# adityaX1412/Experiment-YOLO

Measured on AMD Instinct MI355X. Metric: images/sec (train) DEAL-YOLO-N 640x640 bs=64/GPU, higher is better.
Workload: dtype f16; 1 GPU; DEAL-YOLO-N (yolov8n-ASF-P2P2.yaml) train step 640x640, per-GPU batch 64, fwd+TAL/WIOU+NWD/DFL/BCE loss+bwd+SGD+EMA, BASELINE.json configs[1]; loss_mode=wiou+nwd, settle_steps=18, capture_retries=0, global_batch=64, parallelism=dp1, hipgraph=True

## Files before the change

### experiment-yolo_amd/csrc/tensor_ops.hip

```cpp
#include <cstdlib>
#include "common.h"
#include "dealyolo_hip.h"

static inline int grid_for(long total) {
  long b = (total + 255) / 256;
  if (b > 8192) b = 8192;
  if (b < 1) b = 1;
  return (int)b;
}

__global__ __launch_bounds__(256) void import_image_kernel(const float* x, f16* y, int N, int C, int H, int W, int Cp,
                                                           float mul) {
  const long hw = (long)H * W, total = (long)N * hw;
  for (long pix = (long)blockIdx.x * 256 + threadIdx.x; pix < total; pix += (long)gridDim.x * 256) {
    const long n = pix / hw, r = pix - n * hw;
    for (int c0 = 0; c0 < Cp; c0 += 8) {
      half8 v;
#pragma unroll
      for (int j = 0; j < 8; ++j) v[j] = (c0 + j < C) ? (f16)(x[(n * C + c0 + j) * hw + r] * mul) : (f16)0.f;
      *reinterpret_cast<half8*>(y + pix * Cp + c0) = v;
    }
  }
}
extern "C" int dy_import_image(const float* x, void* y, int n, int c, int h, int w, int cp, float mul,
                               hipStream_t stream) {
  if (cp & 7) return DY_ERR_ALIGN;
  hipLaunchKernelGGL(import_image_kernel, dim3(grid_for((long)n * h * w)), dim3(256), 0, stream, x, (f16*)y, n, c, h, w,
                     cp, mul);
  DY_CHECK_LAUNCH();
  return DY_OK;
}

__global__ __launch_bounds__(256) void import_image_u8_kernel(const unsigned char* x, f16* y, long npix, int Cp) {
  const long quads = npix >> 2;
  for (long q = (long)blockIdx.x * 256 + threadIdx.x; q < quads; q += (long)gridDim.x * 256) {
    const unsigned* p = reinterpret_cast<const unsigned*>(x + q * 12);
    const unsigned w0 = p[0], w1 = p[1], w2 = p[2];
    const unsigned char b[12] = {(unsigned char)w0, (unsigned char)(w0 >> 8), (unsigned char)(w0 >> 16), (unsigned char)(w0 >> 24),
                                 (unsigned char)w1, (unsigned char)(w1 >> 8), (unsigned char)(w1 >> 16), (unsigned char)(w1 >> 24),
                                 (unsigned char)w2, (unsigned char)(w2 >> 8), (unsigned char)(w2 >> 16), (unsigned char)(w2 >> 24)};
#pragma unroll
    for (int k = 0; k < 4; ++k) {
      half8 v;
#pragma unroll
      for (int j = 0; j < 8; ++j) v[j] = j < 3 ? (f16)((float)b[3 * k + j] / 255.f) : (f16)0.f;
      f16* d = y + (q * 4 + k) * Cp;
      *reinterpret_cast<half8*>(d) = v;
      for (int c0 = 8; c0 < Cp; c0 += 8) *reinterpret_cast<half8*>(d + c0) = half8{};
    }
  }
  for (long pix = (quads << 2) + (long)blockIdx.x * 256 + threadIdx.x; pix < npix; pix += (long)gridDim.x * 256) {
    half8 v;
#pragma unroll
    for (int j = 0; j < 8; ++j) v[j] = j < 3 ? (f16)((float)x[pix * 3 + j] / 255.f) : (f16)0.f;
    *reinterpret_cast<half8*>(y + pix * Cp) = v;
    for (int c0 = 8; c0 < Cp; c0 += 8) *reinterpret_cast<half8*>(y + pix * Cp + c0) = half8{};
  }
}
static __device__ __forceinline__ void hsv_jitter(float (&c)[3], float r0, float r1, float r2) {
  const float R = c[0], G = c[1], B = c[2];
  const float V = fmaxf(R, fmaxf(G, B)), mn = fminf(R, fminf(G, B)), d = V - mn;
// ... 308 lines not shown
    const long pix = idx / cpp;
    const int c0 = (int)(idx - pix * cpp) * 8;
    const int x0 = (int)(pix % a.W);
    const long t = pix / a.W;
    const int y0 = (int)(t % a.H);
    const long n = t / a.H;
    float s[8];
#pragma unroll
    for (int j = 0; j < 8; ++j) s[j] = 0.f;
    if (a.accumulate) {
      const half8 o = *reinterpret_cast<const half8*>(a.y + pix * a.ldy + c0);
#pragma unroll
      for (int j = 0; j < 8; ++j) s[j] = (float)o[j];
    }
#pragma unroll
    for (int dy = 0; dy < 5; ++dy) {
      const int wy = y0 - (dy - 2);
      const bool yok = wy >= 0 && wy < a.H;
      const int yc = yok ? wy : y0;
      uint2 raw[5];
      half8 g[5];
      bool ok[5];
#pragma unroll
      for (int dx = 0; dx < 5; ++dx) {
        const int wx = x0 - (dx - 2);
        ok[dx] = yok && wx >= 0 && wx < a.W;
        const long wp = (n * a.H + yc) * a.W + (ok[dx] ? wx : x0);
        raw[dx] = *reinterpret_cast<const uint2*>(a.arg + wp * a.C + c0);
        g[dx] = *reinterpret_cast<const half8*>(a.dy + wp * a.lddy + c0);
      }
#pragma unroll
      for (int dx = 0; dx < 5; ++dx) {
        if (!ok[dx]) continue;
        const uint8_t* ai = reinterpret_cast<const uint8_t*>(&raw[dx]);
        const int code = dy * 5 + dx;
#pragma unroll
        for (int j = 0; j < 8; ++j)
          if (ai[j] == code) s[j] += (float)g[dx][j];
      }
    }
    half8 o;
#pragma unroll
    for (int j = 0; j < 8; ++j) o[j] = (f16)s[j];
    *reinterpret_cast<half8*>(a.y + pix * a.ldy + c0) = o;
  }
}
#define SPPF_THREADS 1024
struct SppfArgs {
  f16* cat;
  uint8_t* arg[3];
  int ld, C, N, H, W, acc[3];
};
template <int CG>
__global__ __launch_bounds__(SPPF_THREADS) void sppf_pool3_fwd_kernel(SppfArgs a) {
  constexpr int G = CG / 8;
  extern __shared__ __attribute__((aligned(16))) char sppf_lds[];
  const int HW = a.H * a.W, items = HW * G;
  half8* cur = reinterpret_cast<half8*>(sppf_lds);
  half8* rowm = cur + items;
  uint2* rowa = reinterpret_cast<uint2*>(rowm + items);
  const int groups = a.C / CG, n = blockIdx.x / groups, c0 = (blockIdx.x - n * groups) * CG;
  f16* const base = a.cat + (size_t)n * HW * a.ld + c0;
  for (int i = threadIdx.x; i < items; i += SPPF_THREADS) {
    const int px = i / G, part = i - px * G;
    cur[i] = *reinterpret_cast<const half8*>(base + (size_t)px * a.ld + part * 8);
  }
  __syncthreads();
  for (int l = 0; l < 3; ++l) {
    for (int i = threadIdx.x; i < items; i += SPPF_THREADS) {
      const int px = i / G, part = i - px * G, y = px / a.W, x = px - y * a.W;
      float best[8];
      uint8_t bd[8];
#pragma unroll
      for (int j = 0; j < 8; ++j) { best[j] = -INFINITY; bd[j] = 0; }
#pragma unroll
      for (int dx = 0; dx < 5; ++dx) {
        const int xx = x + dx - 2;
        if (xx < 0 || xx >= a.W) continue;
        const half8 v = cur[(y * a.W + xx) * G + part];
#pragma unroll
        for (int j = 0; j < 8; ++j) {
          const float f = (float)v[j];
          if (f > best[j] || f != f) { best[j] = f; bd[j] = (uint8_t)dx; }
        }
      }
      half8 o;
#pragma unroll
      for (int j = 0; j < 8; ++j) o[j] = (f16)best[j];
      rowm[i] = o;
      rowa[i] = *reinterpret_cast<const uint2*>(bd);
    }
    __syncthreads();
    f16* const yb = base + (size_t)(l + 1) * a.C;
    uint8_t* const ab = a.arg[l] ? a.arg[l] + (size_t)n * HW * a.C + c0 : nullptr;
    for (int i = threadIdx.x; i < items; i += SPPF_THREADS) {
      const int px = i / G, part = i - px * G, y = px / a.W, x = px - y * a.W;
      float best[8];
      uint8_t bi[8];
#pragma unroll
      for (int j = 0; j < 8; ++j) { best[j] = -INFINITY; bi[j] = 0; }
#pragma unroll
      for (int dy = 0; dy < 5; ++dy) {
        const int yy = y + dy - 2;
        if (yy < 0 || yy >= a.H) continue;
        const int k = (yy * a.W + x) * G + part;
        const half8 v = rowm[k];
        const uint2 ra = rowa[k];
        const uint8_t* rd = reinterpret_cast<const uint8_t*>(&ra);
#pragma unroll
        for (int j = 0; j < 8; ++j) {
          const float f = (float)v[j];
          if (f > best[j] || f != f) { best[j] = f; bi[j] = (uint8_t)(dy * 5 + rd[j]); }
        }
      }
      half8 o;
#pragma unroll
      for (int j = 0; j < 8; ++j) o[j] = (f16)best[j];
      cur[i] = o;
      *reinterpret_cast<half8*>(yb + (size_t)px * a.ld + part * 8) = o;
      if (ab) *reinterpret_cast<uint2*>(ab + (size_t)px * a.C + part * 8) = *reinterpret_cast<const uint2*>(bi);
    }
    __syncthreads();
  }
}
template <int CG>
__global__ __launch_bounds__(SPPF_THREADS) void sppf_pool3_bwd_kernel(SppfArgs a) {
  constexpr int G = CG / 8;
  extern __shared__ __attribute__((aligned(16))) char sppf_lds[];
  const int HW = a.H * a.W, items = HW * G;
  half8* g0 = reinterpret_cast<half8*>(sppf_lds);
  half8* g1 = g0 + items;
  uint2* ar = reinterpret_cast<uint2*>(g1 + items);
  const int groups = a.C / CG, n = blockIdx.x / groups, c0 = (blockIdx.x - n * groups) * CG;
  f16* const base = a.cat + (size_t)n * HW * a.ld + c0;
  for (int i = threadIdx.x; i < items; i += SPPF_THREADS) {
    const int px = i / G, part = i - px * G;
    g0[i] = *reinterpret_cast<const half8*>(base + (size_t)3 * a.C + (size_t)px * a.ld + part * 8);
  }
  for (int l = 2; l >= 0; --l) {
    const uint8_t* const ab = a.arg[l] + (size_t)n * HW * a.C + c0;
    for (int i = threadIdx.x; i < items; i += SPPF_THREADS) {
      const int px = i / G, part = i - px * G;
      ar[i] = *reinterpret_cast<const uint2*>(ab + (size_t)px * a.C + part * 8);
    }
    __syncthreads();
    f16* const tb = base + (size_t)l * a.C;
    for (int i = threadIdx.x; i < items; i += SPPF_THREADS) {
      const int px = i / G, part = i - px * G, y = px / a.W, x = px - y * a.W;
      float s[8];
#pragma unroll
      for (int j = 0; j < 8; ++j) s[j] = 0.f;
      if (a.acc[l]) {
        const half8 o = *reinterpret_cast<const half8*>(tb + (size_t)px * a.ld + part * 8);
#pragma unroll
        for (int j = 0; j < 8; ++j) s[j] = (float)o[j];
      }
#pragma unroll
      for (int dy = 0; dy < 5; ++dy) {
        const int wy = y - (dy - 2);
        if (wy < 0 || wy >= a.H) continue;
#pragma unroll
        for (int dx = 0; dx < 5; ++dx) {
          const int wx = x - (dx - 2);
          if (wx < 0 || wx >= a.W) continue;
          const int k = (wy * a.W + wx) * G + part;
          const uint2 raw = ar[k];
          const half8 g = g0[k];
          const uint8_t* ai = reinterpret_cast<const uint8_t*>(&raw);
          const int code = dy * 5 + dx;
#pragma unroll
          for (int j = 0; j < 8; ++j)
            if (ai[j] == code) s[j] += (float)g[j];
        }
      }
      half8 o;
#pragma unroll
      for (int j = 0; j < 8; ++j) o[j] = (f16)s[j];
      if (l > 0) g1[i] = o;
      else *reinterpret_cast<half8*>(tb + (size_t)px * a.ld + part * 8) = o;
    }
    __syncthreads();
    half8* t = g0; g0 = g1; g1 = t;
  }
}
extern "C" int dy_sppf_pool3_supported(int h, int w, int C) {
  if (h < 1 || w < 1 || C < 8 || (C & 7)) return 0;
  const long px = (long)h * w;
  if (!(C & 15) && px * (2 * 32 + 16) <= 156 * 1024) return 16;
  if (px * (2 * 16 + 8) <= 156 * 1024) return 8;
  return 0;
}
extern "C" int dy_sppf_pool3(void* cat, int ld, int C, void* arg0, void* arg1, void* arg2, int n, int h, int w, hipStream_t stream) {
  const int cg = dy_sppf_pool3_supported(h, w, C);
  if (!cg || !cat || ld < 4 * C) return DY_ERR_ARG;
  if ((ld & 7) || ((uintptr_t)cat & 15)) return DY_ERR_ALIGN;
  SppfArgs a{(f16*)cat, {(uint8_t*)arg0, (uint8_t*)arg1, (uint8_t*)arg2}, ld, C, n, h, w, {0, 0, 0}};
  const size_t lds = (size_t)h * w * (cg / 8) * (2 * 16 + 8);
  static bool attr[2] = {false, false};
  if (cg == 16) {
    if (!attr[0]) { if (hipFuncSetAttribute(reinterpret_cast<const void*>(sppf_pool3_fwd_kernel<16>), hipFuncAttributeMaxDynamicSharedMemorySize, 156 * 1024) != hipSuccess) return DY_ERR_LAUNCH; attr[0] = true; }
    hipLaunchKernelGGL(sppf_pool3_fwd_kernel<16>, dim3(n * (C / 16)), dim3(SPPF_THREADS), lds, stream, a);
  } else {
    if (!attr[1]) { if (hipFuncSetAttribute(reinterpret_cast<const void*>(sppf_pool3_fwd_kernel<8>), hipFuncAttributeMaxDynamicSharedMemorySize, 156 * 1024) != hipSuccess) return DY_ERR_LAUNCH; attr[1] = true; }
    hipLaunchKernelGGL(sppf_pool3_fwd_kernel<8>, dim3(n * (C / 8)), dim3(SPPF_THREADS), lds, stream, a);
  }
  DY_CHECK_LAUNCH();
  return DY_OK;
}
extern "C" int dy_sppf_pool3_backward(void* gcat, int ld, int C, const void* arg0, const void* arg1, const void* arg2, int n, int h,
                                      int w, int acc0, int acc1, int acc2, hipStream_t stream) {
  const int cg = dy_sppf_pool3_supported(h, w, C);
  if (!cg || !gcat || !arg0 || !arg1 || !arg2 || ld < 4 * C) return DY_ERR_ARG;
  if ((ld & 7) || ((uintptr_t)gcat & 15)) return DY_ERR_ALIGN;
  SppfArgs a{(f16*)gcat, {(uint8_t*)arg0, (uint8_t*)arg1, (uint8_t*)arg2}, ld, C, n, h, w, {acc0, acc1, acc2}};
  const size_t lds = (size_t)h * w * (cg / 8) * (2 * 16 + 8);
  static bool attr[2] = {false, false};
  if (cg == 16) {
    if (!attr[0]) { if (hipFuncSetAttribute(reinterpret_cast<const void*>(sppf_pool3_bwd_kernel<16>), hipFuncAttributeMaxDynamicSharedMemorySize, 156 * 1024) != hipSuccess) return DY_ERR_LAUNCH; attr[0] = true; }
    hipLaunchKernelGGL(sppf_pool3_bwd_kernel<16>, dim3(n * (C / 16)), dim3(SPPF_THREADS), lds, stream, a);
  } else {
    if (!attr[1]) { if (hipFuncSetAttribute(reinterpret_cast<const void*>(sppf_pool3_bwd_kernel<8>), hipFuncAttributeMaxDynamicSharedMemorySize, 156 * 1024) != hipSuccess) return DY_ERR_LAUNCH; attr[1] = true; }
    hipLaunchKernelGGL(sppf_pool3_bwd_kernel<8>, dim3(n * (C / 8)), dim3(SPPF_THREADS), lds, stream, a);
  }
  DY_CHECK_LAUNCH();
  return DY_OK;
}

extern "C" int dy_maxpool5(const void* x, int ldx, void* y, int ldy, void* argmax, int n, int h, int w, int C,
                           hipStream_t stream) {
  if ((C & 7) || (ldx & 7) || (ldy & 7)) return DY_ERR_ALIGN;
  PoolArgs a{(const f16*)x, (f16*)y, (uint8_t*)argmax, nullptr, ldx, ldy, 0, C, n, h, w, 0};
  hipLaunchKernelGGL(maxpool5_fwd_kernel, dim3(grid_for((long)n * h * w * (C >> 3))), dim3(256), 0, stream, a);
  DY_CHECK_LAUNCH();
  return DY_OK;
}
extern "C" int dy_maxpool5_backward(const void* dy, int lddy, const void* argmax, void* dx, int lddx, int n, int h,
                                    int w, int C, int accumulate, hipStream_t stream) {
  if ((C & 7) || (lddy & 7) || (lddx & 7)) return DY_ERR_ALIGN;
  PoolArgs a{nullptr, (f16*)dx, (uint8_t*)argmax, (const f16*)dy, 0, lddx, lddy, C, n, h, w, accumulate};
  hipLaunchKernelGGL(maxpool5_bwd_kernel, dim3(grid_for((long)n * h * w * (C >> 3))), dim3(256), 0, stream, a);
  DY_CHECK_LAUNCH();
  return DY_OK;
}

struct SsArgs {
  const f16* r[3];
  int ld[3];
  const f16* res;
  int ldres;
// ... 363 lines not shown
          }
        }
        if (a.mode) *reinterpret_cast<half8*>(a.dr[0] + pos * a.lddr[0] + c0) = o;
      }
      half8 o1;
#pragma unroll
      for (int j = 0; j < 8; ++j) {
        const float tot = gs1[j] + (cpp == 4 ? dpp_read<DY_DPP_ROW_SHL(4)>(gs1[j]) : __shfl_xor(gs1[j], cpp, 64));
        const float xh = ((float)own1[j] - mean[j]) * inv[j];
        if (a.mode == 0) {
          if (!(col & 1)) { ps[j] += tot; px[j] += tot * xh; }
        } else {
          o1[j] = (f16)(sc[j] * (tot - 4.f * mg[j] - 4.f * xh * mgx[j]));
        }
      }
      if (a.mode && !(col & 1)) *reinterpret_cast<half8*>(a.dr[1] + lp1 * a.lddr[1] + c0) = o1;
    }
    half8 o2;
#pragma unroll
    for (int j = 0; j < 8; ++j) {
      float tot;
      if (cpp == 4) {
        tot = gs2[j] + dpp_read<DY_DPP_ROW_SHL(4)>(gs2[j]);
        tot += dpp_read<DY_DPP_ROW_SHL(8)>(tot);
      } else {
        tot = gs2[j] + __shfl_xor(gs2[j], cpp, 64);
        tot += __shfl_xor(tot, 2 * cpp, 64);
      }
      const float xh = ((float)own2[j] - mean[j]) * inv[j];
      if (a.mode == 0) {
        if (!(col & 3)) { ps[j] += tot; px[j] += tot * xh; }
      } else {
        o2[j] = (f16)(sc[j] * (tot - 16.f * mg[j] - 16.f * xh * mgx[j]));
      }
    }
    if (a.mode && !(col & 3)) *reinterpret_cast<half8*>(a.dr[2] + lp2 * a.lddr[2] + c0) = o2;
  }
  if (a.mode == 0) {
    __shared__ float red[2][256][9];
    const int rows = 256 / cpp;
#pragma unroll
    for (int j = 0; j < 8; ++j) {
      red[0][tid][j] = ps[j];
      red[1][tid][j] = px[j];
    }
    __syncthreads();
    for (int i = tid; i < 2 * a.C; i += 256) {
      const int which = i / a.C, c = i - which * a.C, pp = c >> 3, j = c & 7;
      float sum = 0.f;
      for (int r = 0; r < rows; ++r) sum += red[which][r * cpp + pp][j];
      a.partials[((size_t)blockIdx.x * 2 + which) * a.C + c] = sum;
    }
  }
}
extern "C" int dy_scalseq_tail_backward_all(const void* r0, int ld0, const void* r1, int ld1, const void* r2, int ld2,
                                            const void* dy, int lddy, void* dr0, int lddr0, void* dr1, int lddr1,
                                            void* dr2, int lddr2, const float* coef, const float* bwdcoef,
                                            float* partials, int max_partials, int n, int h, int w, int C, int mode,
                                            int* nparts, hipStream_t stream) {
  if ((C & 7) || (C >> 3) > 256 || (h & 3) || (w & 3) || (ld0 & 7) || (ld1 & 7) || (ld2 & 7) || (lddy & 7)) return DY_ERR_ARG;
  if (mode && ((lddr0 & 7) || (lddr1 & 7) || (lddr2 & 7) || !dr0 || !dr1 || !dr2 || !bwdcoef)) return DY_ERR_ARG;
  if (!mode && !partials) return DY_ERR_ARG;
  SsBwdAllArgs a{{(const f16*)r0, (const f16*)r1, (const f16*)r2}, {ld0, ld1, ld2}, (const f16*)dy, lddy,
                 {(f16*)dr0, (f16*)dr1, (f16*)dr2}, {lddr0, lddr1, lddr2}, coef, bwdcoef, partials, C, n, h, w, mode};
  const int rows = 256 / (C >> 3);
  long blocks = ((long)n * (h >> 2) * (w >> 2) + rows - 1) / rows;
  if (blocks > 2048) blocks = 2048;
  if (mode == 0 && blocks > max_partials) blocks = max_partials;
  if (blocks < 1) blocks = 1;
  const int cpp = C >> 3;
  if (cpp <= 16 && 64 % cpp == 0 && w % (64 / cpp) == 0) {
    long wblocks = ((long)n * (h >> 2) * (w / (64 / cpp)) + 3) / 4;
    if (wblocks > 2048) wblocks = 2048;
    if (mode == 0 && wblocks > max_partials) wblocks = max_partials;
    if (wblocks < 1) wblocks = 1;
    if (nparts) *nparts = (int)wblocks;
    hipLaunchKernelGGL(scalseq_bwd_cols_kernel, dim3((int)wblocks), dim3(256), 0, stream, a);
    DY_CHECK_LAUNCH();
    return DY_OK;
  }
  if (nparts) *nparts = (int)blocks;
  hipLaunchKernelGGL(scalseq_bwd_all_kernel, dim3((int)blocks), dim3(256), 0, stream, a);
  DY_CHECK_LAUNCH();
  return DY_OK;
}

__global__ __launch_bounds__(256) void copy_slice_kernel(EwArgs e) {
  const int cpp = e.C >> 3;
  const long total = e.npix * cpp;
  for (long idx = (long)blockIdx.x * 256 + threadIdx.x; idx < total; idx += (long)gridDim.x * 256) {
    const long pix = idx / cpp;
    const int c0 = (int)(idx - pix * cpp) * 8;
    *reinterpret_cast<uint4*>(e.y + pix * e.ldy + c0) = *reinterpret_cast<const uint4*>(e.a + pix * e.lda + c0);
  }
}
extern "C" int dy_copy_slice(const void* x, int ldx, void* y, int ldy, long npix, int C, hipStream_t stream) {
  if ((C & 7) || (ldx & 7) || (ldy & 7)) return DY_ERR_ALIGN;
  EwArgs e{(const f16*)x, nullptr, nullptr, (f16*)y, ldx, 0, 0, ldy, C, npix};
  hipLaunchKernelGGL(copy_slice_kernel, dim3(grid_for(npix * (C >> 3))), dim3(256), 0, stream, e);
  DY_CHECK_LAUNCH();
  return DY_OK;
}
extern "C" int dy_fill_zero(void* p, size_t bytes, hipStream_t stream) {
  return hipMemsetAsync(p, 0, bytes, stream) == hipSuccess ? DY_OK : DY_ERR_LAUNCH;
}

struct ZpArgs {
  const f16* x;
  f16* y;
  const f16* dy;
  f16* dx;
  int ldx, ldy, lddy, lddx, C, N, H, W, accumulate;
};
__global__ __launch_bounds__(256) void zoom_pool_fwd_kernel(ZpArgs a) {
  const int cpp = a.C >> 3;
  const long total = (long)a.N * a.H * a.W * cpp;
  for (long idx = (long)blockIdx.x * 256 + threadIdx.x; idx < total; idx += (long)gridDim.x * 256) {
    const long pix = idx / cpp;
    const int c0 = (int)(idx - pix * cpp) * 8;
    const int ox = (int)(pix % a.W);
    const long t = pix / a.W;
    const int oy = (int)(t % a.H);
    const long n = t / a.H;
    float mx[8], sm[8];
#pragma unroll
    for (int i = 0; i < 4; ++i) {
      const long src = (n * 2 * a.H + 2 * oy + (i >> 1)) * 2 * a.W + 2 * ox + (i & 1);
      const half8 v = *reinterpret_cast<const half8*>(a.x + src * a.ldx + c0);
#pragma unroll
// ... 72 lines not shown
```

### experiment-yolo_amd/ultralytics/hip/__init__.py

```python
from __future__ import annotations

import ctypes as C
import os
import sys

_FLAG = "DEBUG_CLR_GRAPH_PACKET_CAPTURE"


def _hip_already_up():
    t = sys.modules.get("torch")
    try:
        return bool(t is not None and t.cuda.is_initialized())
    except Exception:
        return False


if os.environ.get(_FLAG) is None and not _hip_already_up():
    os.environ[_FLAG] = "0"
GRAPH_SAFE = os.environ.get(_FLAG) == "0"

_HERE = os.path.dirname(os.path.abspath(__file__))
LIB_PATH = os.environ.get("DY_HIP_LIB") or os.path.normpath(os.path.join(_HERE, "..", "..", "csrc", "libdealyolo_hip.so"))

DY_EPI_STATS, DY_EPI_BIAS, DY_EPI_SILU, DY_EPI_F32OUT, DY_EPI_ACCUM, DY_EPI_STATS_ACC = 1, 2, 4, 8, 16, 32
# ... 84 lines not shown
    "dy_refine_select": (i32, [vp, vp, vp, vp, vp, i32, C.c_float, C.c_float, vp, vp, vp]),
    "dy_nms_hard": (i32, [vp, vp, vp, i32, C.c_float, vp, vp]),
    "dy_crop_letterbox_u8_multi": (i32, [vp, vp, vp, vp, vp, vp, i32, i32, vp, vp]),
    "dy_refine_select_multi": (i32, [vp, vp, vp, vp, vp, vp, vp, i32, vp, vp, vp]),
    "dy_two_stage_merge": (i32, [vp, vp, vp, vp, vp, vp, i32, f32, vp, vp, f32, i32, vp, vp, vp, vp]),
    "dy_tile_gather_f32": (i32, [vp, vp, vp, vp, vp, vp, vp, i32, i32, vp, vp]),
    "dy_tile_merge": (i32, [vp, vp, vp, vp, vp, i32, i32, i32, f32, i32, i32, vp, vp, vp, vp, vp]),
    "dy_warp_import_u8": (i32, [vp, vp, vp, i32, i32, i32, vp]),
    "dy_warp_slot_bytes": (i32, []),
    "dy_import_image_u8": (i32, [vp, vp, i32, i32, i32, i32, vp, vp, vp, vp]),
    "dy_add": (i32, [vp, i32, vp, i32, vp, i32, vp, i32, i64, i32, vp]),
    "dy_upsample2x": (i32, [vp, i32, vp, i32, i32, i32, i32, i32, i32, i32, vp]),
    "dy_space_to_depth": (i32, [vp, i32, vp, i32, i32, i32, i32, i32, i32, i32, vp]),
    "dy_maxpool5": (i32, [vp, i32, vp, i32, vp, i32, i32, i32, i32, vp]),
    "dy_maxpool5_backward": (i32, [vp, i32, vp, vp, i32, i32, i32, i32, i32, i32, vp]),
    "dy_bn_group_max": (i32, []),
    "dy_bn_act_apply_acc_split": (i32, [vp, i32, vp, i32, vp, i32, i32, vp, vp, vp, vp, vp, vp, i64, i32, i32, f32, f32, f32, vp]),
    "dy_bn_act_bwd_reduce_acc_split": (i32, [vp, i32, vp, i32, i32, vp, i32, vp, vp, i64, i32, i32, vp]),
    "dy_conv1x1_wgrad_bn_planes": (i32, [C.POINTER(DySegs), vp, i32, vp, vp, i32, i32, vp, i32, vp, vp, vp, vp, vp, f32, vp, vp, i32, i32, i32,
                                         i32, i32, i32, vp]),
    "dy_conv1x1_wgrad_dgrad_supported": (i32, [i32, i32, i32, i32, i32]),
    "dy_wgrad_dgrad_kernel_name": (i32, [i32, i32, i32, i32, i32, i32, C.c_char_p, i32]),
    "dy_conv1x1_wgrad_dgrad_bn": (i32, [vp, i32, vp, i32, vp, i32, vp, vp, vp, vp, f32, vp, vp, vp, vp, i32, i32, i32, i32, i32, i32, i32, i32, vp]),
    "dy_conv1x1_wgrad_dgrad_bn_segs": (i32, [C.POINTER(DySegs), vp, i32, vp, i32, vp, vp, vp, vp, f32, vp, vp, vp, C.POINTER(DySegs), i32, i32,
                                             i32, i32, i32, i32, vp]),
    "dy_conv1x1_wgrad_dgrad_bn_planes": (i32, [C.POINTER(DySegs), vp, i32, vp, vp, i32, i32, vp, i32, vp, vp, vp, vp, f32, vp, vp, vp, vp, i32, i32,
                                               C.POINTER(DySegs), i32, i32, i32, i32, i32, i32, vp]),
    "dy_conv1x1_dgrad_bn_supported": (i32, [i32, i32, i32, i32, i32]),
    "dy_dgrad_only_kernel_name": (i32, [i32, i32, i32, i32, i32, i32, C.c_char_p, i32]),
    "dy_conv1x1_dgrad_bn": (i32, [vp, vp, i32, i32, vp, i32, vp, vp, f32, vp, vp, i32, i32, C.POINTER(DySegs), i32, i32, i32, i32, i32, vp]),
    "dy_bn_act_apply_acc_group": (i32, [i32, vp, vp, vp, vp, vp, vp, vp, vp, vp, vp, vp, vp, vp, vp, vp, vp]),
    "dy_bn_act_bwd_reduce_acc_group": (i32, [i32, vp, vp, vp, vp, vp, vp, vp, vp, vp]),
    "dy_bn_act_bwd_reduce_rows": (i32, [vp, i32, vp, i32, vp, vp, i32, i32, i32, i32, vp, i32, i32, vp]),
    "dy_head_box_decode": (i32, [vp, i32, vp, vp, vp, vp, i32, i32, i32, i32, i32, i32, i32, vp]),
    "dy_cls_head_supported": (i32, [i32, i32]),
    "dy_cls_head_slabs": (i32, []),
    "dy_cls_head_forward": (i32, [vp, i32, vp, vp, vp, vp, i64, i32, i32, vp]),
    "dy_cls_head_backward": (i32, [vp, i32, vp, vp, vp, vp, i32, i32, vp, vp, i64, i32, i32, vp]),
    "dy_head_box_decode_levels": (i32, [i32, vp, vp, vp, vp, vp, vp, i32, vp, i32, vp, vp, i32, i32, vp]),
    "dy_conv1x1_rows_backward_levels": (i32, [i32, vp, vp, vp, vp, vp, vp, i32, vp, vp, vp, vp, vp, vp, vp, i32, vp, vp, i32, i32, vp]),
    "dy_cls_head_forward_levels": (i32, [i32, vp, vp, vp, vp, vp, vp, vp, i32, i32, vp]),
    "dy_cls_head_backward_levels": (i32, [i32, vp, vp, vp, vp, vp, vp, vp, vp, vp, vp, vp, i32, i32, vp]),
    "dy_conv1x1_rows_supported": (i32, [i32, i32]),
    "dy_conv1x1_rows_slabs": (i32, [i32, i32, i32]),
    "dy_conv1x1_rows_backward": (i32, [vp, i32, vp, vp, i32, vp, i32, i32, vp, vp, i32, i32, vp, vp, i32, i32, i32, i32, i32, vp]),
    "dy_sppf_pool3_supported": (i32, [i32, i32, i32]),
    "dy_sppf_pool3": (i32, [vp, i32, i32, vp, vp, vp, i32, i32, i32, vp]),
    "dy_sppf_pool3_backward": (i32, [vp, i32, i32, vp, vp, vp, i32, i32, i32, i32, i32, i32, vp]),
    "dy_scalseq_tail": (i32, [vp, i32, vp, i32, vp, i32, vp, i32, vp, i32, vp, i32, i32, i32, i32, vp]),
    "dy_scalseq_tail_backward": (i32, [vp, i32, vp, i32, vp, i32, vp, i32, vp, i32, vp, vp, vp, i32, i32, i32, i32, i32,
                                       i32, i32, ip, vp]),
    "dy_scalseq_tail_backward_all": (i32, [vp, i32, vp, i32, vp, i32, vp, i32, vp, i32, vp, i32, vp, i32, vp, vp, vp, i32, i32,
                                           i32, i32, i32, i32, ip, vp]),
    "dy_zoom_pool": (i32, [vp, i32, vp, i32, i32, i32, i32, i32, vp]),
    "dy_zoom_pool_backward": (i32, [vp, i32, vp, i32, vp, i32, i32, i32, i32, i32, i32, vp]),
    "dy_copy_slice": (i32, [vp, i32, vp, i32, i64, i32, vp]),
    "dy_fill_zero": (i32, [vp, sz, vp]),
    "dy_loss_workspace_bytes": (sz, [i32, i32, i32]),
    "dy_loss_workspace_layout": (i32, [i32, i32, i32, C.POINTER(sz), C.POINTER(sz), C.POINTER(sz)]),
    "dy_detection_loss": (i32, [C.POINTER(DyLossArgs), vp]),
    "dy_tal_assign": (i32, [vp, ip, ip, C.POINTER(f32), i32, i32, i32, i32, i32, vp, vp, vp, vp, vp, vp, vp, vp]),
    "dy_head_infer_supported": (i32, [i32, i32, i32, i32]),
    "dy_head_infer_levels": (i32, [i32, vp, vp, vp, vp, vp, vp, vp, vp, vp, vp, vp, i32, i32, i32, vp, vp]),
    "dy_head_infer_levels_logits": (i32, [i32, vp, vp, vp, vp, vp, vp, vp, vp, vp, vp, vp, i32, i32, i32, vp, vp, vp, vp]),
    "dy_decode_predictions": (i32, [vp, vp, ip, ip, C.POINTER(f32), i32, i32, i32, i32, vp, vp]),
    "dy_nms_candidates": (i32, [vp, i32, i32, i32, f32, i32, vp, i32, vp, vp, vp, vp, i32, vp]),
    "dy_nms_presort_workspace": (sz, [i32, i32]),
    "dy_nms_presort": (i32, [vp, vp, vp, vp, i32, i32, i32, vp, vp, vp, vp, vp]),
    "dy_soft_nms": (i32, [vp, vp, vp, vp, vp, vp, vp, vp, i32, i32, f32, f32, f32, f32, vp]),
    "dy_set_hyper": (i32, [vp, vp, vp]),
    "dy_optimizer_step": (i32, [vp, vp, vp, vp, vp, i64, i64, i64, vp, vp, vp, i64, vp, vp, vp, i32, vp]),
    "dy_optimizer_step_seg": (i32, [vp, vp, vp, vp, vp, i64, lp, vp, vp, vp, i64, vp, vp, vp, i32, vp]),
    "dy_axpy_f32": (i32, [vp, vp, f32, i64, vp]),
    "dy_scale_img": (i32, [vp, i32, i32, i32, i32, i32, i32, i32, i32, vp, vp]),
    "dy_tta_merge": (i32, [i32, C.POINTER(vp), ip, ip, ip, C.POINTER(f32), ip, i32, i32, i32, i32, vp, vp]),
    "dy_bootstrap_ap": (i32, [vp, vp, vp, vp, vp, i32, i32, i32, i32, vp, vp, vp]),
    "dy_confusion_matrix": (i32, [vp, vp, i32, vp, vp, vp, i32, vp, i32, i32, i32, i32, f32, f32, i32, vp, vp, vp]),
    "dy_count_fp": (i32, [vp, vp, vp, vp, vp, i32, f32, C.c_double, vp, vp, vp]),
}

_LIB = None


def lib():
    global _LIB
    if _LIB is None:
        if not os.path.exists(LIB_PATH):
            raise RuntimeError(
                f"{LIB_PATH} not found. The DEAL-YOLO hot path has no CPU/PyTorch fallback: build the HIP library "
                f"first (python -c 'import __graft_entry__ as g; g.build()' or `make -C experiment-yolo_amd/csrc`).")
        L = C.CDLL(LIB_PATH)
        for name, (res, args) in SIGNATURES.items():
            fn = getattr(L, name)
            fn.restype, fn.argtypes = res, args
        if L.dy_segs_bytes() != C.sizeof(DySegs):
            raise RuntimeError(f"{LIB_PATH} lays DySegs out in {L.dy_segs_bytes()} bytes, this binding in {C.sizeof(DySegs)}: rebuild the library")
        if L.dy_loss_args_bytes() != C.sizeof(DyLossArgs):
            raise RuntimeError(f"{LIB_PATH} was built with a DyLossArgs of {L.dy_loss_args_bytes()} bytes, this binding lays out "
                               f"{C.sizeof(DyLossArgs)}: rebuild the library (make -C experiment-yolo_amd/csrc)")
        _LIB = L
    return _LIB


def check(rc, name):
    if rc != 0:
        raise RuntimeError(f"{name} failed: {_ERR.get(rc, rc)}")
# ... 1 lines not shown
```

### include/dealyolo_hip.h

```cpp
#ifndef DEALYOLO_HIP_H
#define DEALYOLO_HIP_H

#include <stddef.h>
#include <stdint.h>

#ifdef __cplusplus
extern "C" {
#endif

#ifndef __HIP__
typedef struct ihipStream_t* hipStream_t;
#endif

#define DY_OK 0
#define DY_ERR_ARG (-1)
#define DY_ERR_LAUNCH (-2)
#define DY_ERR_ALIGN (-3)
#define DY_ERR_CAPACITY (-4)

#define DY_MAX_SEGS 8
typedef struct DySegs {
  int nseg;
  int c_end[DY_MAX_SEGS];
  int ld[DY_MAX_SEGS];
// ... 127 lines not shown
                    int C, int act, hipStream_t stream);
int dy_bn_act_apply_acc(const void* x, int ldx, const void* res, int ldr, void* y, int ldy, const double* acc,
                        const float* gamma, const float* beta, float* running_mean, float* running_var, float* coef,
                        long npix, int C, int act, float count, float eps, float momentum, hipStream_t stream);
int dy_bn_act_bwd_reduce_acc(const void* dy, int lddy, const void* x, int ldx, const float* coef, double* acc, long npix,
                             int C, int act, void* res_grad, int ldrg, int res_accumulate, hipStream_t stream);
int dy_bn_group_max(void);
int dy_bn_act_apply_acc_group(int n, const void* const* x, const int* ldx, void* const* y, const int* ldy, const double* const* acc,
                              const float* const* gamma, const float* const* beta, float* const* running_mean, float* const* running_var,
                              float* const* coef, const long* npix, const int* C, const float* count, const float* eps,
                              const float* momentum, hipStream_t stream);
int dy_bn_act_bwd_reduce_acc_group(int n, const void* const* dy, const int* lddy, const void* const* x, const int* ldx,
                                   const float* const* coef, double* const* acc, const long* npix, const int* C, hipStream_t stream);
int dy_bn_act_bwd_reduce_rows(const void* dy, int lddy, const void* x, int ldx, const float* coef, double* acc, int n, int hw, int C,
                              int act, const int* assigned, int A, int a0, hipStream_t stream);
int dy_bn_act_bwd_apply_acc(const void* dy, int lddy, const void* x, int ldx, void* dx, int lddx, const float* coef,
                            const double* acc, float* dgamma, float* dbeta, long npix, int C, int act, float count,
                            hipStream_t stream);
int dy_bn_act_bwd_reduce(const void* dy, int lddy, const void* x, int ldx, const float* coef, float* partials,
                         int max_partials, long npix, int C, int act, int* nparts, hipStream_t stream);
int dy_bn_bwd_finalize(const float* partials, int nparts, float* dgamma, float* dbeta, float* bwdcoef, int C,
                       float count, int accumulate, hipStream_t stream);
int dy_bn_act_bwd_apply(const void* dy, int lddy, const void* x, int ldx, void* dx, int lddx, const float* coef,
                        const float* bwdcoef, long npix, int C, int act, int frozen_stats, hipStream_t stream);

int dy_import_image(const float* x_nchw, void* y, int n, int c, int h, int w, int cp, float mul, hipStream_t stream);
int dy_import_image_u8(const void* x, void* y, int n, int h, int w, int cp, const void* flip, const int* index,
                       const float* hsv, hipStream_t stream);
int dy_warp_import_u8(const void* pool, const void* slots, void* y, int n, int s, int cp, hipStream_t stream);
int dy_warp_slot_bytes(void);
int dy_add(const void* a, int lda, const void* b, int ldb, const void* c, int ldc, void* y, int ldy, long npix, int C,
           hipStream_t stream);
int dy_upsample2x(const void* x, int ldx, void* y, int ldy, int n, int h, int w, int C, int backward, int accumulate,
                  hipStream_t stream);
int dy_space_to_depth(void* x, int ldx, void* y, int ldy, int n, int h, int w, int C, int backward, int accumulate,
                      hipStream_t stream);
int dy_maxpool5(const void* x, int ldx, void* y, int ldy, void* argmax, int n, int h, int w, int C, hipStream_t stream);
int dy_maxpool5_backward(const void* dy, int lddy, const void* argmax, void* dx, int lddx, int n, int h, int w, int C,
                         int accumulate, hipStream_t stream);
int dy_sppf_pool3_supported(int h, int w, int C);
int dy_sppf_pool3(void* cat, int ld, int C, void* arg0, void* arg1, void* arg2, int n, int h, int w, hipStream_t stream);
int dy_sppf_pool3_backward(void* gcat, int ld, int C, const void* arg0, const void* arg1, const void* arg2, int n, int h, int w,
                           int acc0, int acc1, int acc2, hipStream_t stream);
int dy_scalseq_tail(const void* r0, int ld0, const void* r1, int ld1, const void* r2, int ld2, const void* res,
                    int ldres, void* y, int ldy, const float* coef, int n, int h, int w, int C, hipStream_t stream);
int dy_scalseq_tail_backward(const void* r0, int ld0, const void* r1, int ld1, const void* r2, int ld2, const void* dy,
                             int lddy, void* dr, int lddr, const float* coef, const float* bwdcoef, float* partials,
                             int max_partials, int n, int h, int w, int C, int level, int mode, int* nparts,
                             hipStream_t stream);
int dy_scalseq_tail_backward_all(const void* r0, int ld0, const void* r1, int ld1, const void* r2, int ld2,
                                 const void* dy, int lddy, void* dr0, int lddr0, void* dr1, int lddr1, void* dr2,
                                 int lddr2, const float* coef, const float* bwdcoef, float* partials, int max_partials,
                                 int n, int h, int w, int C, int mode, int* nparts, hipStream_t stream);
int dy_zoom_pool(const void* x, int ldx, void* y, int ldy, int n, int h, int w, int C, hipStream_t stream);
int dy_zoom_pool_backward(const void* x, int ldx, const void* dy, int lddy, void* dx, int lddx, int n, int h, int w, int C,
                          int accumulate, hipStream_t stream);
int dy_copy_slice(const void* x, int ldx, void* y, int ldy, long npix, int C, hipStream_t stream);
int dy_fill_zero(void* p, size_t bytes, hipStream_t stream);

typedef struct DyLossArgs {
  int nl, B, nc, ncp, nmax;
  const float* box[4];
  const float* cls[4];
  void* dbox[4];
  void* dcls[4];
  int H[4], W[4];
  float stride[4];
  const float* t_batch_idx;
  const float* t_cls;
  const float* t_boxes;
  int n_targets;
  const int* n_targets_dev;
  float img_w, img_h;
  float hyp_box, hyp_cls, hyp_dfl;
  int use_wiou, use_nwd;
  float iou_ratio;
  const float* gscale;
  float* scalars;
  void* workspace;
  int dbox_rows_only;
  int box_from_input;
  const void* box_in[4];
  int box_in_ld[4];
  const float* box_w[4];
  const float* box_b[4];
  const float* box_in_coef[4];
  int box_family;
  int box_ltype;
  int box_fm;
  int box_modifier;
  float inner_ratio;
  float focaler_d, focaler_u;
  float shape_scale;
  float piou_lambda;
} DyLossArgs;
#define DY_BOX_FAMILY_LEGACY 0
#define DY_BOX_FAMILY_WISE 1
#define DY_BOX_FAMILY_BBOX 2
#define DY_BOX_IOU 0
#define DY_BOX_WIOU 1
#define DY_BOX_EIOU 2
#define DY_BOX_GIOU 3
#define DY_BOX_DIOU 4
#define DY_BOX_CIOU 5
#define DY_BOX_SIOU 6
#define DY_BOX_SHAPEIOU 7
// ... 115 lines not shown
```

Measured before the change: 6089 images/s.

## Add integer-key SPPF pooling and persistent grid-capped ScalSeq backward kernels

```diff
diff --git a/experiment-yolo_amd/csrc/tensor_ops.hip b/experiment-yolo_amd/csrc/tensor_ops.hip
--- a/experiment-yolo_amd/csrc/tensor_ops.hip
+++ b/experiment-yolo_amd/csrc/tensor_ops.hip
@@ -7,6 +7,10 @@
   if (b > 8192) b = 8192;
   if (b < 1) b = 1;
   return (int)b;
+}
+static bool tensor_ops_v1() {
+  const char* e = getenv("DY_TENSOR_OPS_V1");
+  return e && e[0] == '1' && !e[1];
 }
 
 __global__ __launch_bounds__(256) void import_image_kernel(const float* x, f16* y, int N, int C, int H, int W, int Cp,
@@ -421,9 +425,8 @@
   int ld, C, N, H, W, acc[3];
 };
 template <int CG>
-__global__ __launch_bounds__(SPPF_THREADS) void sppf_pool3_fwd_kernel(SppfArgs a) {
+static __device__ __forceinline__ void sppf_pool3_fwd_body(const SppfArgs& a, char* sppf_lds) {
   constexpr int G = CG / 8;
-  extern __shared__ __attribute__((aligned(16))) char sppf_lds[];
   const int HW = a.H * a.W, items = HW * G;
   half8* cur = reinterpret_cast<half8*>(sppf_lds);
   half8* rowm = cur + items;
@@ -488,6 +491,106 @@
       cur[i] = o;
       *reinterpret_cast<half8*>(yb + (size_t)px * a.ld + part * 8) = o;
       if (ab) *reinterpret_cast<uint2*>(ab + (size_t)px * a.C + part * 8) = *reinterpret_cast<const uint2*>(bi);
+    }
+    __syncthreads();
+  }
+}
+template <int CG>
+__global__ __launch_bounds__(SPPF_THREADS) void sppf_pool3_fwd_kernel(SppfArgs a) {
+  extern __shared__ __attribute__((aligned(16))) char sppf_lds[];
+  sppf_pool3_fwd_body<CG>(a, sppf_lds);
+}
+template <int CG>
+__global__ __launch_bounds__(SPPF_THREADS) void sppf_pool3_fwd_v2_kernel(SppfArgs a) {
+  constexpr int G = CG / 8;
+  constexpr unsigned KNINF = 0x03ffu;
+  extern __shared__ __attribute__((aligned(16))) char sppf_lds[];
+  const int HW = a.H * a.W, items = HW * G;
+  uint4* cur = reinterpret_cast<uint4*>(sppf_lds);
+  uint4* row0 = cur + items;
+  uint4* row1 = row0 + items;
+  int* special = reinterpret_cast<int*>(row1 + items);
+  const int groups = a.C / CG, n = blockIdx.x / groups, c0 = (blockIdx.x - n * groups) * CG;
+  f16* const base = a.cat + (size_t)n * HW * a.ld + c0;
+  if (threadIdx.x == 0) *special = 0;
+  __syncthreads();
+  bool bad = false;
+  for (int i = threadIdx.x; i < items; i += SPPF_THREADS) {
+    const int px = i / G, part = i - px * G;
+    const uint4 v = *reinterpret_cast<const uint4*>(base + (size_t)px * a.ld + part * 8);
+    const unsigned w[4] = {v.x, v.y, v.z, v.w};
+    unsigned k[4];
+#pragma unroll
+    for (int d = 0; d < 4; ++d) {
+      const unsigned lo = w[d] & 0xffffu, hi = w[d] >> 16;
+      bad |= (lo & 0x7fffu) > 0x7c00u || lo == 0x8000u || (hi & 0x7fffu) > 0x7c00u || hi == 0x8000u;
+      k[d] = w[d] ^ ((((w[d] >> 15) & 0x00010001u) * 0xffffu) | 0x80008000u);
+    }
+    cur[i] = uint4{k[0], k[1], k[2], k[3]};
+  }
+  if (bad) *special = 1;
+  __syncthreads();
+  if (*special) {
+    __syncthreads();
+    sppf_pool3_fwd_body<CG>(a, sppf_lds);
+    return;
+  }
+  for (int l = 0; l < 3; ++l) {
+    for (int i = threadIdx.x; i < items; i += SPPF_THREADS) {
+      const int px = i / G, part = i - px * G, y = px / a.W, x = px - y * a.W;
+      unsigned best[8];
+#pragma unroll
+      for (int dx = 0; dx < 5; ++dx) {
+        const int xx = min(max(x + dx - 2, 0), a.W - 1);
+        const unsigned t = (unsigned)(63 - xx);
+        const uint4 v = cur[(y * a.W + xx) * G + part];
+        const unsigned w[4] = {v.x, v.y, v.z, v.w};
+#pragma unroll
+        for (int d = 0; d < 4; ++d) {
+          const unsigned lo = (w[d] << 16) | t, hi = (w[d] & 0xffff0000u) | t;
+          best[2 * d] = dx ? max(best[2 * d], lo) : lo;
+          best[2 * d + 1] = dx ? max(best[2 * d + 1], hi) : hi;
+        }
+      }
+      const int kx = (63 - y) * 5 + x - 61, ninf = (63 - y) * 5 + 4;
+      unsigned o[8];
+#pragma unroll
+      for (int j = 0; j < 8; ++j) {
+        const unsigned low = (best[j] >> 16) == KNINF ? (unsigned)ninf : (unsigned)((int)(best[j] & 0xffffu) + kx);
+        o[j] = (best[j] & 0xffff0000u) | low;
+      }
+      row0[i] = uint4{o[0], o[1], o[2], o[3]};
+      row1[i] = uint4{o[4], o[5], o[6], o[7]};
+    }
+    __syncthreads();
+    f16* const yb = base + (size_t)(l + 1) * a.C;
+    uint8_t* const ab = a.arg[l] ? a.arg[l] + (size_t)n * HW * a.C + c0 : nullptr;
+    for (int i = threadIdx.x; i < items; i += SPPF_THREADS) {
+      const int px = i / G, part = i - px * G, y = px / a.W, x = px - y * a.W;
+      unsigned best[8];
+#pragma unroll
+      for (int dy = 0; dy < 5; ++dy) {
+        const int yy = min(max(y + dy - 2, 0), a.H - 1);
+        const int k = (yy * a.W + x) * G + part;
+        const uint4 v0 = row0[k], v1 = row1[k];
+        const unsigned w[8] = {v0.x, v0.y, v0.z, v0.w, v1.x, v1.y, v1.z, v1.w};
+#pragma unroll
+        for (int j = 0; j < 8; ++j) best[j] = dy ? max(best[j], w[j]) : w[j];
+      }
+      const unsigned ky = (unsigned)(329 - 5 * y);
+      unsigned kp[4], hv[4], code[8];
+#pragma unroll
+      for (int j = 0; j < 8; ++j) code[j] = (best[j] >> 16) == KNINF ? 0u : (ky - (best[j] & 0xffffu)) & 0xffu;
+#pragma unroll
+      for (int d = 0; d < 4; ++d) {
+        kp[d] = (best[2 * d + 1] & 0xffff0000u) | (best[2 * d] >> 16);
+        hv[d] = kp[d] ^ ((((~kp[d] >> 15) & 0x00010001u) * 0xffffu) | 0x80008000u);
+      }
+      cur[i] = uint4{kp[0], kp[1], kp[2], kp[3]};
+      *reinterpret_cast<uint4*>(yb + (size_t)px * a.ld + part * 8) = uint4{hv[0], hv[1], hv[2], hv[3]};
+      if (ab)
+        *reinterpret_cast<uint2*>(ab + (size_t)px * a.C + part * 8) =
+            uint2{code[0] | code[1] << 8 | code[2] << 16 | code[3] << 24, code[4] | code[5] << 8 | code[6] << 16 | code[7] << 24};
     }
     __syncthreads();
   }
@@ -564,6 +667,19 @@
   if (!cg || !cat || ld < 4 * C) return DY_ERR_ARG;
   if ((ld & 7) || ((uintptr_t)cat & 15)) return DY_ERR_ALIGN;
   SppfArgs a{(f16*)cat, {(uint8_t*)arg0, (uint8_t*)arg1, (uint8_t*)arg2}, ld, C, n, h, w, {0, 0, 0}};
+  const size_t lds2 = (size_t)h * w * (cg / 8) * 48 + 16;
+  if (!tensor_ops_v1() && h <= 63 && w <= 63 && lds2 <= 156 * 1024) {
+    static bool attr2[2] = {false, false};
+    if (cg == 16) {
+      if (!attr2[0]) { if (hipFuncSetAttribute(reinterpret_cast<const void*>(sppf_pool3_fwd_v2_kernel<16>), hipFuncAttributeMaxDynamicSharedMemorySize, 156 * 1024) != hipSuccess) return DY_ERR_LAUNCH; attr2[0] = true; }
+      hipLaunchKernelGGL(sppf_pool3_fwd_v2_kernel<16>, dim3(n * (C / 16)), dim3(SPPF_THREADS), lds2, stream, a);
+    } else {
+      if (!attr2[1]) { if (hipFuncSetAttribute(reinterpret_cast<const void*>(sppf_pool3_fwd_v2_kernel<8>), hipFuncAttributeMaxDynamicSharedMemorySize, 156 * 1024) != hipSuccess) return DY_ERR_LAUNCH; attr2[1] = true; }
+      hipLaunchKernelGGL(sppf_pool3_fwd_v2_kernel<8>, dim3(n * (C / 8)), dim3(SPPF_THREADS), lds2, stream, a);
+    }
+    DY_CHECK_LAUNCH();
+    return DY_OK;
+  }
   const size_t lds = (size_t)h * w * (cg / 8) * (2 * 16 + 8);
   static bool attr[2] = {false, false};
   if (cg == 16) {
@@ -1033,6 +1149,169 @@
       a.partials[((size_t)blockIdx.x * 2 + which) * a.C + c] = sum;
     }
   }
+}
+static __device__ __forceinline__ half8 ld16(const f16* sbase, unsigned voff) {
+  return *reinterpret_cast<const half8*>(reinterpret_cast<const char*>(sbase) + voff);
+}
+static __device__ __forceinline__ void st16(f16* sbase, unsigned voff, uint4 v) {
+  *reinterpret_cast<uint4*>(reinterpret_cast<char*>(sbase) + voff) = v;
+}
+static __device__ __forceinline__ void mul_to_f16(int hi, unsigned& pk, float a, float b) {
+  if (hi) asm("v_fma_mixhi_f16 %0, %1, %2, 0" : "+v"(pk) : "v"(a), "v"(b));
+  else asm("v_fma_mixlo_f16 %0, %1, %2, 0" : "+v"(pk) : "v"(a), "v"(b));
+}
+template <int CPP, int MODE>
+__global__ __launch_bounds__(256, 4) void scalseq_bwd_v2_kernel(SsBwdAllArgs a, int nvb) {
+#pragma clang fp contract(off)
+  constexpr int PW = 64 / CPP, ROWS = 256 / CPP, CC = CPP * 8;
+  const int h1 = a.H >> 1, w1 = a.W >> 1, h2 = a.H >> 2, w2 = a.W >> 2;
+  const int tid = threadIdx.x, lane = tid & 63;
+  const int wave = __builtin_amdgcn_readfirstlane(tid >> 6);
+  const int part = lane % CPP, col = lane / CPP, c0 = part * 8;
+  __shared__ float cf[6][CC];
+  if (tid < CC) {
+#pragma unroll
+    for (int k = 0; k < 4; ++k) cf[k][tid] = a.coef[k * CC + tid];
+    cf[4][tid] = MODE ? a.bwdcoef[tid] : 0.f;
+    cf[5][tid] = MODE ? a.bwdcoef[CC + tid] : 0.f;
+  }
+  __syncthreads();
+  float ps[8], px[8];
+  const unsigned vo0 = (unsigned)(col * a.ld[0] + c0) * 2u, vody = (unsigned)(col * a.lddy + c0) * 2u;
+  const unsigned vo1 = (unsigned)((col >> 1) * a.ld[1] + c0) * 2u, vo2 = (unsigned)((col >> 2) * a.ld[2] + c0) * 2u;
+  const unsigned vd0 = MODE ? (unsigned)(col * a.lddr[0] + c0) * 2u : 0u, vd1 = MODE ? (unsigned)((col >> 1) * a.lddr[1] + c0) * 2u : 0u;
+  const unsigned vd2 = MODE ? (unsigned)((col >> 2) * a.lddr[2] + c0) * 2u : 0u;
+  const unsigned chunks = (unsigned)(a.W / PW);
+  const unsigned items = (unsigned)a.N * (unsigned)h2 * chunks;
+  const unsigned nv = MODE ? gridDim.x : (unsigned)nvb;
+  __shared__ float red[MODE ? 1 : 2][MODE ? 1 : 256][9];
+  for (unsigned vb = blockIdx.x; vb < nv; vb += gridDim.x) {
+#pragma unroll
+    for (int j = 0; j < 8; ++j) ps[j] = px[j] = 0.f;
+    for (unsigned it = vb * 4 + (unsigned)wave; it < items; it += nv * 4) {
+      const unsigned xc = it % chunks, t = it / chunks;
+      const int y2 = (int)(t % (unsigned)h2);
+      const long n = (long)(t / (unsigned)h2);
+      const long x0 = (long)(xc * PW);
+      const long lp2 = (n * h2 + y2) * w2 + (x0 >> 2);
+      long lp1[2], pos[4];
+      half8 own2, own1[2], own0[4], g[4];
+      unsigned pk0[4][4] = {}, pk1[2][4] = {}, pk2[4] = {};
+      int coff = c0;
+      asm volatile("" : "+v"(coff));
+      const float* const cp = &cf[0][0] + coff;
+      float sc[8], sh[8], mean[8], inv[8], mg[8], mgx[8];
+#pragma unroll
+      for (int j = 0; j < 8; ++j) {
+        sc[j] = cp[j]; sh[j] = cp[CC + j]; mean[j] = cp[2 * CC + j]; inv[j] = cp[3 * CC + j];
+        mg[j] = MODE ? cp[4 * CC + j] : 0.f; mgx[j] = MODE ? cp[5 * CC + j] : 0.f;
+      }
+      own2 = ld16(a.r[2] + lp2 * a.ld[2], vo2);
+#pragma unroll
+      for (int hf = 0; hf < 2; ++hf) {
+        lp1[hf] = (n * h1 + (y2 * 2 + hf)) * w1 + (x0 >> 1);
+        own1[hf] = ld16(a.r[1] + lp1[hf] * a.ld[1], vo1);
+      }
+#pragma unroll
+      for (int q = 0; q < 4; ++q) {
+        pos[q] = (n * a.H + (y2 * 4 + q)) * a.W + x0;
+        own0[q] = ld16(a.r[0] + pos[q] * a.ld[0], vo0);
+        g[q] = ld16(a.dy + pos[q] * a.lddy, vody);
+      }
+      asm volatile("" : "+v"(own2), "+v"(own1[0]), "+v"(own1[1]), "+v"(own0[0]), "+v"(own0[1]), "+v"(own0[2]), "+v"(own0[3]), "+v"(g[0]), "+v"(g[1]),
+                        "+v"(g[2]), "+v"(g[3]));
+#pragma unroll
+      for (int j = 0; j < 8; ++j) {
+        const float zz2 = __builtin_fmaf((float)own2[j], sc[j], sh[j]);
+        const float z2 = zz2 > 0.f ? zz2 : 0.1f * zz2;
+        float gs2 = 0.f;
+#pragma unroll
+        for (int hf = 0; hf < 2; ++hf) {
+          const float zz1 = __builtin_fmaf((float)own1[hf][j], sc[j], sh[j]);
+          const float z1 = zz1 > 0.f ? zz1 : 0.1f * zz1;
+          float gs1 = 0.f;
+#pragma unroll
+          for (int rr = 0; rr < 2; ++rr) {
+            const int q = hf * 2 + rr;
+            const float zz0 = __builtin_fmaf((float)own0[q][j], sc[j], sh[j]);
+            const float z0 = zz0 > 0.f ? zz0 : 0.1f * zz0;
+            int am = 0;
+            float zb = z0;
+            if (z1 > zb) { am = 1; zb = z1; }
+            if (z2 > zb) { am = 2; zb = z2; }
+            const float gg = (float)g[q][j] * (zb > 0.f ? 1.f : 0.1f);
+            const float g0 = am == 0 ? gg : 0.f;
+            gs1 += am == 1 ? gg : 0.f;
+            gs2 += am == 2 ? gg : 0.f;
+            const float xh0 = ((float)own0[q][j] - mean[j]) * inv[j];
+            if (MODE == 0) {
+              ps[j] += g0;
+              px[j] = __builtin_fmaf(xh0, g0, px[j]);
+            } else {
+              mul_to_f16(j & 1, pk0[q][j >> 1], sc[j], __builtin_fmaf(-mgx[j], xh0, g0 - mg[j]));
+            }
+          }
+          const float tot = gs1 + (CPP == 4 ? dpp_read<DY_DPP_ROW_SHL(4)>(gs1) : __shfl_xor(gs1, CPP, 64));
+          const float xh = ((float)own1[hf][j] - mean[j]) * inv[j];
+          if (MODE == 0) {
+            if (!(col & 1)) { ps[j] += tot; px[j] = __builtin_fmaf(xh, tot, px[j]); }
+          } else {
+            mul_to_f16(j & 1, pk1[hf][j >> 1], sc[j], __builtin_fmaf(mgx[j], -4.f * xh, tot - 4.f * mg[j]));
+          }
+        }
+        float tot;
+        if (CPP == 4) {
+          tot = gs2 + dpp_read<DY_DPP_ROW_SHL(4)>(gs2);
+          tot += dpp_read<DY_DPP_ROW_SHL(8)>(tot);
+        } else {
+          tot = gs2 + __shfl_xor(gs2, CPP, 64);
+          tot += __shfl_xor(tot, 2 * CPP, 64);
+        }
+        const float xh = ((float)own2[j] - mean[j]) * inv[j];
+        if (MODE == 0) {
+          if (!(col & 3)) { ps[j] += tot; px[j] = __builtin_fmaf(xh, tot, px[j]); }
+        } else {
+          mul_to_f16(j & 1, pk2[j >> 1], sc[j], __builtin_fmaf(mgx[j], -16.f * xh, tot - 16.f * mg[j]));
+        }
+      }
+      if (MODE) {
+#pragma unroll
+        for (int q = 0; q < 4; ++q) st16(a.dr[0] + pos[q] * a.lddr[0], vd0, uint4{pk0[q][0], pk0[q][1], pk0[q][2], pk0[q][3]});
+        if (!(col & 1)) {
+#pragma unroll
+          for (int hf = 0; hf < 2; ++hf) st16(a.dr[1] + lp1[hf] * a.lddr[1], vd1, uint4{pk1[hf][0], pk1[hf][1], pk1[hf][2], pk1[hf][3]});
+        }
+        if (!(col & 3)) st16(a.dr[2] + lp2 * a.lddr[2], vd2, uint4{pk2[0], pk2[1], pk2[2], pk2[3]});
+      }
+    }
+    if constexpr (MODE == 0) {
+#pragma unroll
+      for (int j = 0; j < 8; ++j) {
+        red[0][tid][j] = ps[j];
+        red[1][tid][j] = px[j];
+      }
+      __syncthreads();
+      if (tid < 2 * CC) {
+        const int which = tid / CC, c = tid - which * CC, pp = c >> 3, j = c & 7;
+        float sum = 0.f;
+#pragma unroll 16
+        for (int r = 0; r < ROWS; ++r) sum += red[which][r * CPP + pp][j];
+        a.partials[((size_t)vb * 2 + which) * CC + c] = sum;
+      }
+      __syncthreads();
+    }
+  }
+}
+static int g_scalseq_grid_cap = 0;
+extern "C" int dy_scalseq_bwd_grid_cap(int cap) {
+  const int old = g_scalseq_grid_cap;
+  g_scalseq_grid_cap = cap > 0 ? cap : 0;
+  return old;
+}
+template <int CPP>
+static void scalseq_v2_launch(const SsBwdAllArgs& a, int mode, int nvb, int grid, hipStream_t stream) {
+  if (mode) hipLaunchKernelGGL((scalseq_bwd_v2_kernel<CPP, 1>), dim3(grid), dim3(256), 0, stream, a, nvb);
+  else hipLaunchKernelGGL((scalseq_bwd_v2_kernel<CPP, 0>), dim3(grid), dim3(256), 0, stream, a, nvb);
 }
 extern "C" int dy_scalseq_tail_backward_all(const void* r0, int ld0, const void* r1, int ld1, const void* r2, int ld2,
                                             const void* dy, int lddy, void* dr0, int lddr0, void* dr1, int lddr1,
@@ -1056,6 +1335,20 @@
     if (mode == 0 && wblocks > max_partials) wblocks = max_partials;
     if (wblocks < 1) wblocks = 1;
     if (nparts) *nparts = (int)wblocks;
+    const long items = (long)n * (h >> 2) * (w / (64 / cpp));
+    if (!tensor_ops_v1() && items < (1L << 31) - 4 * 2048) {
+      const int cap = g_scalseq_grid_cap ? g_scalseq_grid_cap : DY_NUM_CUS * 4;
+      const int grid = wblocks < cap ? (int)wblocks : cap;
+      switch (cpp) {
+        case 1: scalseq_v2_launch<1>(a, mode, (int)wblocks, grid, stream); break;
+        case 2: scalseq_v2_launch<2>(a, mode, (int)wblocks, grid, stream); break;
+        case 4: scalseq_v2_launch<4>(a, mode, (int)wblocks, grid, stream); break;
+        case 8: scalseq_v2_launch<8>(a, mode, (int)wblocks, grid, stream); break;
+        default: scalseq_v2_launch<16>(a, mode, (int)wblocks, grid, stream); break;
+      }
+      DY_CHECK_LAUNCH();
+      return DY_OK;
+    }
     hipLaunchKernelGGL(scalseq_bwd_cols_kernel, dim3((int)wblocks), dim3(256), 0, stream, a);
     DY_CHECK_LAUNCH();
     return DY_OK;
diff --git a/experiment-yolo_amd/ultralytics/hip/__init__.py b/experiment-yolo_amd/ultralytics/hip/__init__.py
--- a/experiment-yolo_amd/ultralytics/hip/__init__.py
+++ b/experiment-yolo_amd/ultralytics/hip/__init__.py
@@ -160,6 +160,7 @@
                                        i32, i32, ip, vp]),
     "dy_scalseq_tail_backward_all": (i32, [vp, i32, vp, i32, vp, i32, vp, i32, vp, i32, vp, i32, vp, i32, vp, vp, vp, i32, i32,
                                            i32, i32, i32, i32, ip, vp]),
+    "dy_scalseq_bwd_grid_cap": (i32, [i32]),
     "dy_zoom_pool": (i32, [vp, i32, vp, i32, i32, i32, i32, i32, vp]),
     "dy_zoom_pool_backward": (i32, [vp, i32, vp, i32, vp, i32, i32, i32, i32, i32, i32, vp]),
     "dy_copy_slice": (i32, [vp, i32, vp, i32, i64, i32, vp]),
diff --git a/include/dealyolo_hip.h b/include/dealyolo_hip.h
--- a/include/dealyolo_hip.h
+++ b/include/dealyolo_hip.h
@@ -203,6 +203,7 @@
                                  const void* dy, int lddy, void* dr0, int lddr0, void* dr1, int lddr1, void* dr2,
                                  int lddr2, const float* coef, const float* bwdcoef, float* partials, int max_partials,
                                  int n, int h, int w, int C, int mode, int* nparts, hipStream_t stream);
+int dy_scalseq_bwd_grid_cap(int cap);
 int dy_zoom_pool(const void* x, int ldx, void* y, int ldy, int n, int h, int w, int C, hipStream_t stream);
 int dy_zoom_pool_backward(const void* x, int ldx, const void* dy, int lddy, void* dx, int lddx, int n, int h, int w, int C,
                           int accumulate, hipStream_t stream);
```

New measurement: 6162 images/s (median of 6 runs). 1.01x the previous value.
